# WhatAShot/Electrocardio-Panorama

Measured on AMD Instinct MI355X. Metric: ECG-samples/sec (train step), higher is better.
Workload: dtype f32 (conv products: fp32 operands split into fp16 hi+lo = 22-23 bits, block-scaled, 3 fp16 matrix products each, fp32 accumulate; fp32-class, not IEEE fp32)

## Files before the change

### electrocardio_panorama_amd/csrc/elementwise.hip

```cpp
#include "nef_common.h"
#include "roi_unpool.h"

namespace {

__global__ void chscale_fwd_kernel(const float* __restrict__ x, const float* __restrict__ s, int64_t s_bs,
                                   float* __restrict__ y, int B, int C, int T) {
    const int64_t rows = (int64_t)B * C;
    const int wave = threadIdx.x >> 6, lane = threadIdx.x & 63;
    for (int64_t row = (int64_t)blockIdx.x * 4 + wave; row < rows; row += (int64_t)gridDim.x * 4) {
        const int b = (int)(row / C), c = (int)(row % C);
        const float f = s[(int64_t)b * s_bs + c];
        const float* xr = x + row * T;
        float* yr = y + row * T;
        for (int t = lane; t < T; t += 64) yr[t] = xr[t] * f;
    }
}

__global__ void chscale_bwd_kernel(const float* __restrict__ gy, const float* __restrict__ x,
                                   const float* __restrict__ s, int64_t s_bs, float* __restrict__ gx,
                                   float* __restrict__ gs, int B, int C, int T, int relu_x) {
    const int64_t rows = (int64_t)B * C;
    const int wave = threadIdx.x >> 6, lane = threadIdx.x & 63;
    for (int64_t row = (int64_t)blockIdx.x * 4 + wave; row < rows; row += (int64_t)gridDim.x * 4) {
        const int b = (int)(row / C), c = (int)(row % C);
// ... 145 lines not shown
            lat[t] = m0;
            lat[t + 64] = m1;
            d0[t] = f * m0;
            d0[t + 64] = f * m1;
            d0[pass + t] = f * p0;
            d0[pass + t + 64] = f * p1;
        }
        for (; t < TW; t += 64) {
            vec s = src[t];
            vec pk = s;
            for (int v = 1; v < V; ++v) {
                const vec x = src[(int64_t)v * lead + t];
                s += x;
                if (v == cp) pk = x;
            }
            const vec m = s / fv;
            lat[t] = m;
            d0[t] = f * m;
            d0[pass + t] = f * pk;
        }
    }
}

__global__ __launch_bounds__(256) void lead_mean_mix_shared_pair_kernel(const float* __restrict__ z1, const float* __restrict__ z2r,
                                                                        const float* __restrict__ q, float* __restrict__ latent,
                                                                        float* __restrict__ D2, int B, int V, int T, int c1, int c2,
                                                                        const int32_t* __restrict__ choice_dev, int cshift) {
    typedef float vec __attribute__((ext_vector_type(4)));
    if (choice_dev) { c1 = choice_dev[0]; c2 = choice_dev[1]; }
    const int64_t pairs = (int64_t)B * 128;
    const int pshift = cshift - 1;
    const int64_t nidx = (int64_t)B << pshift;
    const int wave = threadIdx.x >> 6, lane = threadIdx.x & 63;
    const float fv = (float)V;
    const int TW = T / 2;
    const int mid = T / 4;
    const int64_t pass = pairs * TW;
    const int64_t lead = (int64_t)128 * T / 4;
    for (int64_t idx = (int64_t)blockIdx.x * 4 + wave; idx < nidx; idx += (int64_t)gridDim.x * 4) {
        const int64_t pr = ((idx >> pshift) << 7) | (idx & ((1 << pshift) - 1));
        const int64_t row = 2 * pr;
        const int b = (int)(row >> 8), c = (int)(row & 255);
        const vec* src = (const vec*)((c < 128 ? z1 : z2r) + ((int64_t)b * V * 128 + (c & 127)) * T);
        const int cp = c < 128 ? c1 : c2;
        const float f0 = q[row], f1 = q[row + 1];
        vec* lat = (vec*)latent + pr * TW;
        vec* d0 = (vec*)D2 + pr * TW;
        int t = lane;
        for (; t + 64 < TW; t += 128) {
            vec s0 = src[t], s1 = src[t + 64];
            vec p0 = s0, p1 = s1;
            for (int v = 1; v < V; ++v) {
                const vec x0 = src[(int64_t)v * lead + t], x1 = src[(int64_t)v * lead + t + 64];
                s0 += x0;
                s1 += x1;
                if (v == cp) { p0 = x0; p1 = x1; }
            }
            const vec m0 = s0 / fv, m1 = s1 / fv;
            const vec g0 = t < mid ? vec{f0, f0, f0, f0} : (t > mid ? vec{f1, f1, f1, f1} : vec{f0, f0, f1, f1});
            const vec g1 = t + 64 < mid ? vec{f0, f0, f0, f0} : (t + 64 > mid ? vec{f1, f1, f1, f1} : vec{f0, f0, f1, f1});
            lat[t] = m0;
            lat[t + 64] = m1;
            d0[t] = g0 * m0;
            d0[t + 64] = g1 * m1;
            d0[pass + t] = g0 * p0;
            d0[pass + t + 64] = g1 * p1;
        }
        for (; t < TW; t += 64) {
            vec sm = src[t];
            vec pk = sm;
            for (int v = 1; v < V; ++v) {
                const vec x = src[(int64_t)v * lead + t];
                sm += x;
                if (v == cp) pk = x;
            }
            const vec m = sm / fv;
            const vec g0 = t < mid ? vec{f0, f0, f0, f0} : (t > mid ? vec{f1, f1, f1, f1} : vec{f0, f0, f1, f1});
            lat[t] = m;
            d0[t] = g0 * m;
            d0[pass + t] = g0 * pk;
        }
    }
}

__device__ __forceinline__ float up2_bwd_edge(const float* __restrict__ gr, int Tin, int m) {
    const int To = 2 * Tin;
    float s = 0.f;
#pragma unroll
    for (int d = -1; d <= 2; ++d) {
        const int i = 2 * m + d;
        if (i < 0 || i >= To) continue;
        float src = 0.5f * ((float)i + 0.5f) - 0.5f;
        if (src < 0.f) src = 0.f;
        int i0 = (int)src;
        if (i0 > Tin - 1) i0 = Tin - 1;
        const int i1 = i0 + (i0 < Tin - 1 ? 1 : 0);
        const float l1 = src - (float)i0;
        const float l0 = 1.f - l1;
        const float g = gr[i];
        if (i0 == m) s += l0 * g;
        if (i1 == m) s += l1 * g;
    }
    return s;
}

// ... 76 lines not shown
            } else {
                ga = g0[t]; gb = g0[gpass + t]; gc = SHARED ? 0.f : g0[2 * gpass + t];
            }
            const float g_pick = SHARED ? gb : (first ? gb : gc);
            const float g_mean = SHARED ? ga : (first ? (ga + gc) : (ga + gb));
            const float l = lat[t];
            const float pk = zsrc[(int64_t)pick_v * 128 * T + t];
            acc += g_mean * l + g_pick * pk;
            const float gm = f * g_mean / fv;
            for (int v = 0; v < V; ++v) {
                float o = gm + (v == pick_v ? f * g_pick : 0.f);
                if (relu_z1 && first && !(zsrc[(int64_t)v * 128 * T + t] > 0.f)) o = 0.f;
                gdst[(int64_t)v * 128 * T + t] = o;
            }
        }
        acc = nef_wave_sum(acc);
        if (lane == 0) gq[row] = acc;
    }
}

constexpr int MIX_RS_MAX_V = 4;

template <int NV>
__global__ __launch_bounds__(256) void mix_bwd_shared_pair_kernel(const float* __restrict__ gD, const float* __restrict__ latent,
                                                                  const float* __restrict__ z1, const float* __restrict__ z2r,
                                                                  const float* __restrict__ q, float* __restrict__ gz1,
                                                                  float* __restrict__ gz2r, float* __restrict__ gq, int B, int V, int T,
                                                                  int c1, int c2, const int32_t* __restrict__ choice_dev, int relu_z1,
                                                                  int cshift, double* __restrict__ rowsum) {
    typedef float vec __attribute__((ext_vector_type(4)));
    if (choice_dev) { c1 = choice_dev[0]; c2 = choice_dev[1]; }
    const int64_t pairs = (int64_t)B * 128;
    const int pshift = cshift - 1;
    const int64_t nidx = (int64_t)B << pshift;
    const int wave = threadIdx.x >> 6, lane = threadIdx.x & 63;
    const float fv = (float)V;
    const int TW = T / 2, mid = T / 4;
    const int64_t gpass = pairs * TW;
    const int64_t lead = (int64_t)128 * T / 4;
    for (int64_t idx = (int64_t)blockIdx.x * 4 + wave; idx < nidx; idx += (int64_t)gridDim.x * 4) {
        const int64_t pr = ((idx >> pshift) << 7) | (idx & ((1 << pshift) - 1));
        const int64_t row = 2 * pr;
        const int b = (int)(row >> 8), c = (int)(row & 255);
        const bool first = c < 128;
        const int pick_v = first ? c1 : c2;
        const float f0 = q[row], f1 = q[row + 1];
        const vec* lat = (const vec*)latent + pr * TW;
        const vec* zsrc = (const vec*)((first ? z1 : z2r) + ((int64_t)b * V * 128 + (c & 127)) * T);
        vec* gdst = (vec*)((first ? gz1 : gz2r) + ((int64_t)b * V * 128 + (c & 127)) * T);
        const vec* g0 = (const vec*)gD + pr * TW;
        const vec* g1r = g0 + gpass;
        const bool mask = relu_z1 && first;
        float acc0 = 0.f, acc1 = 0.f;
        double rs0[NV > 0 ? NV : 1], rs1[NV > 0 ? NV : 1];
#pragma unroll
        for (int v = 0; v < NV; ++v) rs0[v] = rs1[v] = 0.0;
        for (int t = lane; t < TW; t += 64) {
            const vec ga = g0[t], gb = g1r[t], l4 = lat[t], pk = zsrc[(int64_t)pick_v * lead + t];
            const vec fq = t < mid ? vec{f0, f0, f0, f0} : (t > mid ? vec{f1, f1, f1, f1} : vec{f0, f0, f1, f1});
#pragma unroll
            for (int e = 0; e < 4; ++e) {
                const float term = ga[e] * l4[e] + gb[e] * pk[e];
                if (t < mid || (t == mid && e < 2)) acc0 += term; else acc1 += term;
// ... 18 lines not shown
                        const vec o = one_lead(v);
                        const double lo = (double)o[0] + (double)o[1], hi = (double)o[2] + (double)o[3];
                        if (t < mid) rs0[v] += lo + hi;
                        else if (t > mid) rs1[v] += lo + hi;
                        else { rs0[v] += lo; rs1[v] += hi; }
                    }
            } else {
                for (int v = 0; v < V; ++v) one_lead(v);
            }
        }
        acc0 = nef_wave_sum(acc0);
        acc1 = nef_wave_sum(acc1);
        if (lane == 0) { gq[row] = acc0; gq[row + 1] = acc1; }
        if constexpr (NV > 0) {
            double* const rdst = rowsum + (int64_t)b * V * 128 + (c & 127);
#pragma unroll
            for (int v = 0; v < NV; ++v)
                if (v < V) {
                    const double a0 = nef_wave_sum_d(rs0[v]), a1 = nef_wave_sum_d(rs1[v]);
                    if (lane == 0) { rdst[v * 128] = a0; rdst[v * 128 + 1] = a1; }
                }
        }
    }
}

__device__ __forceinline__ float up2_at(const float* __restrict__ xr, int Tin, int i) {
    float src = 0.5f * ((float)i + 0.5f) - 0.5f;
    if (src < 0.f) src = 0.f;
    int i0 = (int)src;
    if (i0 > Tin - 1) i0 = Tin - 1;
    const int i1 = i0 + (i0 < Tin - 1 ? 1 : 0);
    const float l1 = src - (float)i0;
    const float l0 = 1.f - l1;
    return l0 * xr[i0] + l1 * xr[i1];
}

__global__ void upsample2_fwd_kernel(const float* __restrict__ x, float* __restrict__ y, int64_t N, int Tin) {
    const int To = 2 * Tin;
    const int wave = threadIdx.x >> 6, lane = threadIdx.x & 63;
    for (int64_t row = (int64_t)blockIdx.x * 4 + wave; row < N; row += (int64_t)gridDim.x * 4) {
        const float* xr = x + row * Tin;
        float* yr = y + row * To;
        for (int i = lane; i < To; i += 64) yr[i] = up2_at(xr, Tin, i);
    }
}

// ... 1965 lines not shown
                           q, latent, D2, B, V, T, c1, c2, choice_dev, cshift);
    else if (T % 2 == 0)
        hipLaunchKernelGGL(lead_mean_mix_shared_kernel<2>, grid, dim3(256), 0, st, z1, z2r, q, latent, D2, B, V, T, c1, c2, choice_dev,
                           cshift);
    else
        hipLaunchKernelGGL(lead_mean_mix_shared_kernel<1>, grid, dim3(256), 0, st, z1, z2r, q, latent, D2, B, V, T, c1, c2, choice_dev,
                           cshift);
}

int nef_lead_mean_mix_shared(const float* z1, const float* z2r, const float* q, float* latent, float* D2, int B, int V,
                             int T, int c1, int c2, const int32_t* choice_dev, nef_stream_t stream) {
    NEF_ENTER();
    NEF_REQUIRE(z1 && z2r && q && latent && D2, NEF_E_NULL);
    NEF_REQUIRE(B > 0 && V > 0 && T > 0 && c1 >= 0 && c1 < V && c2 >= 0 && c2 < V, NEF_E_SHAPE);
    lead_mean_mix_shared_launch(z1, z2r, q, latent, D2, B, V, T, c1, c2, choice_dev, 8, NEF_ST);
    return nef_launch_status();
}

int nef_lead_mean_mix_unpool(const float* z1, const float* z2b, const int64_t* rois, const float* q, float* latent, float* D2,
                             int32_t* status, int B, int V, int T, int c1, int c2, const int32_t* choice_dev, nef_stream_t stream) {
    NEF_ENTER();
    NEF_REQUIRE(z1 && z2b && rois && q && latent && D2, NEF_E_NULL);
    NEF_REQUIRE(B > 0 && V > 0 && V <= NEF_UNPOOL_MIX_MAX_V && T > 0 && c1 >= 0 && c1 < V && c2 >= 0 && c2 < V, NEF_E_SHAPE);
    lead_mean_mix_shared_launch(z1, nullptr, q, latent, D2, B, V, T, c1, c2, choice_dev, 7, NEF_ST);
    nef_unpool_mix_fwd_z2(z2b, rois, q, latent, D2, status, B, V, T, c2, choice_dev, NEF_ST);
    return nef_launch_status();
}

int nef_mix_bwd(const float* gD, const float* latent, const float* z1, const float* z2r, const float* q, float* gz1,
                float* gz2r, float* gq, int B, int V, int T, int c1, int c2, const int32_t* choice_dev, int relu_z1, int up,
                int shared, nef_stream_t stream) {
    NEF_ENTER();
    NEF_REQUIRE(gD && latent && z1 && z2r && q && gz1 && gz2r && gq, NEF_E_NULL);
    NEF_REQUIRE(B > 0 && V > 0 && T > (shared ? 1 : 0) && c1 >= 0 && c1 < V && c2 >= 0 && c2 < V, NEF_E_SHAPE);
    const bool al16 = (((uintptr_t)gD | (uintptr_t)latent | (uintptr_t)z1 | (uintptr_t)z2r | (uintptr_t)gz1 | (uintptr_t)gz2r) & 15) == 0;
#define NEF_MIX_BWD(UP, SHARED)                                                                                                \
    hipLaunchKernelGGL((mix_bwd_kernel<UP, SHARED>), dim3(nef_stream_grid((int64_t)B * 256, 4)), dim3(256), 0, NEF_ST, gD, latent, \
                       z1, z2r, q, gz1, gz2r, gq, B, V, T, c1, c2, choice_dev, relu_z1, 8)
    if (shared && !up && T % 4 == 2 && T >= 8 && al16)
        hipLaunchKernelGGL(mix_bwd_shared_pair_kernel<0>, dim3(nef_stream_grid((int64_t)B * 128, 4)), dim3(256), 0, NEF_ST, gD, latent, z1,
                           z2r, q, gz1, gz2r, gq, B, V, T, c1, c2, choice_dev, relu_z1, 8, (double*)nullptr);
    else if (shared && up) NEF_MIX_BWD(true, true);
    else if (shared) NEF_MIX_BWD(false, true);
    else if (up) NEF_MIX_BWD(true, false);
    else NEF_MIX_BWD(false, false);
#undef NEF_MIX_BWD
    return nef_launch_status();
}

static int mix_bwd_unpool_launch(const float* gD, const float* latent, const float* z1, const float* z2b, const int64_t* rois, const float* q,
                                 float* gz1, float* gz2b, float* gq, int B, int V, int T, int c1, int c2, const int32_t* choice_dev,
                                 int relu_z1, float* gz1_chan_sum, void* ws, size_t ws_bytes, int* in_kernel, nef_stream_t stream) {
    NEF_REQUIRE(gD && latent && z1 && z2b && rois && q && gz1 && gz2b && gq, NEF_E_NULL);
    NEF_REQUIRE(B > 0 && V > 0 && T > 1 && T <= NEF_UNPOOL_MIX_MAX_T && c1 >= 0 && c1 < V && c2 >= 0 && c2 < V, NEF_E_SHAPE);
    const bool al16 = (((uintptr_t)gD | (uintptr_t)latent | (uintptr_t)z1 | (uintptr_t)gz1) & 15) == 0;
    const bool pair = T % 4 == 2 && T >= 8 && al16;
    const bool rs = gz1_chan_sum && pair && V <= MIX_RS_MAX_V;
    if (in_kernel) *in_kernel = rs;
#define NEF_MIX_PAIR(NV, ROWSUM)                                                                                                        \
    hipLaunchKernelGGL(mix_bwd_shared_pair_kernel<NV>, dim3(nef_stream_grid((int64_t)B * 64, 4)), dim3(256), 0, NEF_ST, gD, latent, z1, \
                       (const float*)nullptr, q, gz1, (float*)nullptr, gq, B, V, T, c1, c2, choice_dev, relu_z1, 7, ROWSUM)
    if (rs) {
        NEF_MIX_PAIR(MIX_RS_MAX_V, (double*)ws);
        hipLaunchKernelGGL(rowsum_to_channel, dim3(128 * V), dim3(256), 0, NEF_ST, (const double*)ws, gz1_chan_sum, B, 128 * V);
    } else if (pair)
        NEF_MIX_PAIR(0, (double*)nullptr);
    else
        hipLaunchKernelGGL((mix_bwd_kernel<false, true>), dim3(nef_stream_grid((int64_t)B * 128, 4)), dim3(256), 0, NEF_ST, gD, latent, z1,
                           (const float*)nullptr, q, gz1, (float*)nullptr, gq, B, V, T, c1, c2, choice_dev, relu_z1, 7);
#undef NEF_MIX_PAIR
    nef_unpool_mix_bwd_z2(gD, latent, z2b, rois, q, gz2b, gq, B, V, T, c2, choice_dev, pair ? 4 : ((T & 1) == 0 && T >= 8 ? 2 : 1), NEF_ST);
    if (gz1_chan_sum && !rs)
        return nef_chan_sum(gz1, gz1_chan_sum, ws, ws_bytes, B, 128 * V, T, stream);
    return nef_launch_status();
}

int nef_mix_bwd_unpool(const float* gD, const float* latent, const float* z1, const float* z2b, const int64_t* rois, const float* q,
                       float* gz1, float* gz2b, float* gq, int B, int V, int T, int c1, int c2, const int32_t* choice_dev, int relu_z1,
                       nef_stream_t stream) {
    NEF_ENTER();
    return mix_bwd_unpool_launch(gD, latent, z1, z2b, rois, q, gz1, gz2b, gq, B, V, T, c1, c2, choice_dev, relu_z1, nullptr, nullptr, 0,
                                 nullptr, stream);
}

size_t nef_mix_bwd_unpool_rs_ws_bytes(int B, int V) {
    if (B <= 0 || V <= 0) return 0;
    const size_t rows = (size_t)B * 128 * V * sizeof(double), cs = nef_chan_sum_ws_bytes(128 * V);
    return rows > cs ? rows : cs;
}

int nef_mix_bwd_unpool_rs(const float* gD, const float* latent, const float* z1, const float* z2b, const int64_t* rois, const float* q,
                          float* gz1, float* gz2b, float* gq, float* gz1_chan_sum, void* ws, size_t ws_bytes, int* in_kernel, int B, int V,
                          int T, int c1, int c2, const int32_t* choice_dev, int relu_z1, nef_stream_t stream) {
    NEF_ENTER();
// ... 579 lines not shown
```

### electrocardio_panorama_amd/csrc/roi.hip

```cpp
#include "nef_common.h"
#include "roi_unpool.h"

namespace {

using namespace nef_unpool;

__device__ __forceinline__ float grid_x(const int64_t* __restrict__ roi_b, int j, int s, int T) {
    const float sc = (float)(2.0 / (double)T);
    const float r0 = ((float)roi_b[2 * j] * 0.25f) * sc + (-1.0f);
    const float r1 = ((float)roi_b[2 * j + 1] * 0.25f) * sc + (-1.0f);
    const float step = (r1 - r0) / (float)(BINS - 1);
    return s < BINS / 2 ? r0 + step * (float)s : r1 - step * (float)(BINS - 1 - s);
}

__device__ __forceinline__ float col_weight(float gx) {
    const float ix = ((gx + 1.f) * 1.f - 1.f) * 0.5f;
    const float x0 = floorf(ix);
    const float we = ix - x0;
    const float ww = 1.f - we;
    float w = 0.f;
    if (x0 == 0.f) w += ww;
    if (x0 + 1.f == 0.f) w += we;
    return w;
}
// ... 121 lines not shown
            constexpr int NU = 20;
            for (int t0 = 0; t0 < T; t0 += 64 * NU) {
                float v[NU];
#pragma unroll
                for (int u = 0; u < NU; ++u) v[u] = (t0 + u * 64 + lane < T) ? grow[t0 + u * 64 + lane] : 0.f;
#pragma unroll
                for (int u = 0; u < NU; ++u)
                    if (t0 + u * 64 + lane < T) strip[t0 + u * 64 + lane] = v[u];
            }
            __builtin_amdgcn_fence(__ATOMIC_RELEASE, "wavefront");
            __builtin_amdgcn_wave_barrier();
            gr = strip;
        }
        float* gz = gzseg + row * NSEG * SEGW;
        float acc[(NSEG + 1) / 2] = {0.f, 0.f, 0.f, 0.f};
        unpool_gather_row(gr, st, lane, acc);
#pragma unroll
        for (int k = 0; k < (NSEG + 1) / 2; ++k)
            if (2 * k + half < NSEG) gz[(2 * k + half) * SEGW + s] = acc[k];
        if constexpr (STAGED) __builtin_amdgcn_wave_barrier();
    }
}

__device__ __forceinline__ bool segment_of(const SegTable& st, int t, int& i, float& sc, int& jb) {
    int off = st.off[0];
    sc = st.scale[0];
    jb = 0;
#pragma unroll
    for (int j = 1; j < NSEG; ++j)
        if (t >= st.off[j]) { off = st.off[j]; sc = st.scale[j]; jb = j * SEGW; }
    i = t - off;
    return t < st.off[NSEG - 1] + st.len[NSEG - 1];
}

template <int W>
__global__ __launch_bounds__(256) void unpool_mix_fwd_z2_kernel(const float* __restrict__ z2b, const int64_t* __restrict__ rois,
                                                                const float* __restrict__ q, float* __restrict__ latent,
                                                                float* __restrict__ D2, int32_t* __restrict__ status, int B, int V,
                                                                int T, int c2, const int32_t* __restrict__ choice_dev) {
    typedef float vec __attribute__((ext_vector_type(W)));
    extern __shared__ float strip_lds[];
    constexpr int ROW = NSEG * SEGW;
    if (choice_dev) c2 = choice_dev[1];
    const int64_t rows = (int64_t)B * 128;
    const int wave = __builtin_amdgcn_readfirstlane((int)(threadIdx.x >> 6)), lane = threadIdx.x & 63;
    const int64_t per_wave = (rows + (int64_t)gridDim.x * 4 - 1) / ((int64_t)gridDim.x * 4);
    const int64_t row_lo = ((int64_t)blockIdx.x * 4 + wave) * per_wave;
    const int64_t row_hi = row_lo + per_wave < rows ? row_lo + per_wave : rows;
    float* strip = strip_lds + wave * V * ROW;
    const int n = V * ROW;
    const float fv = (float)V;
    const int64_t pass = (int64_t)B * 256 * T;
    int b_cur = -1;
    SegTable st;
    for (int64_t row = row_lo; row < row_hi; ++row) {
        const int b = (int)(row >> 7), c = (int)(row & 127);
        if (b != b_cur) {
            b_cur = b;
            const bool ok = load_segments(rois + (int64_t)b * NSEG * 2, T, st);
            if (!ok && status && lane == 0) status[0] = 1;
        }
        const float* zr = z2b + ((int64_t)b * V * 128 + c) * ROW;
        constexpr int NU = 8;
        for (int e0 = 0; e0 < n; e0 += 64 * NU) {
            float r[NU];
#pragma unroll
            for (int u = 0; u < NU; ++u) {
                const int e = e0 + u * 64 + lane, v = e / ROW;
                r[u] = e < n ? zr[(int64_t)v * 128 * ROW + (e - v * ROW)] : 0.f;
            }
#pragma unroll
            for (int u = 0; u < NU; ++u)
                if (e0 + u * 64 + lane < n) strip[e0 + u * 64 + lane] = r[u];
        }
        __builtin_amdgcn_fence(__ATOMIC_RELEASE, "wavefront");
        __builtin_amdgcn_wave_barrier();
        const int64_t orow = ((int64_t)b * 256 + 128 + c) * T;
        const float f = q[b * 256 + 128 + c];
        for (int p = lane; p < T / W; p += 64) {
            vec m, dm, dp;
#pragma unroll
            for (int w = 0; w < W; ++w) {
                int i, jb;
                float sc;
                const bool in = segment_of(st, W * p + w, i, sc, jb);
                int i0 = 0, i1 = 0;
                float l0 = 0.f, l1 = 0.f;
                if (in) lerp_src(i, sc, i0, i1, l0, l1);
                float sum = 0.f, pk = 0.f;
                for (int v = 0; v < V; ++v) {
                    const float val = in ? unpool_lerp(l0, strip[v * ROW + jb + i0], l1, strip[v * ROW + jb + i1]) : 0.f;
                    sum = v == 0 ? val : sum + val;
                    if (v == 0 || v == c2) pk = val;
                }
                const float mean = sum / fv;
                m[w] = mean;
                dm[w] = f * mean;
                dp[w] = f * pk;
            }
            *(vec*)(latent + orow + W * p) = m;
            *(vec*)(D2 + orow + W * p) = dm;
            *(vec*)(D2 + pass + orow + W * p) = dp;
        }
        __builtin_amdgcn_wave_barrier();
    }
}

template <int G>
__global__ __launch_bounds__(256) void unpool_mix_bwd_z2_kernel(const float* __restrict__ gD, const float* __restrict__ latent,
                                                                const float* __restrict__ z2b, const int64_t* __restrict__ rois,
                                                                const float* __restrict__ q, float* __restrict__ gz2b,
                                                                float* __restrict__ gq, int B, int V, int T, int c2,
                                                                const int32_t* __restrict__ choice_dev) {
    extern __shared__ float strip_lds[];
    constexpr int ROW = NSEG * SEGW;
    if (choice_dev) c2 = choice_dev[1];
    const int64_t rows = (int64_t)B * 128;
    const int wave = __builtin_amdgcn_readfirstlane((int)(threadIdx.x >> 6)), lane = threadIdx.x & 63;
    const int s = lane & (SEGW - 1), half = lane >> 5;
    const int64_t per_wave = (rows + (int64_t)gridDim.x * 4 - 1) / ((int64_t)gridDim.x * 4);
    const int64_t row_lo = ((int64_t)blockIdx.x * 4 + wave) * per_wave;
    const int64_t row_hi = row_lo + per_wave < rows ? row_lo + per_wave : rows;
    float* sa = strip_lds + wave * (2 * T + ROW);
    float* sb = sa + T;
    float* pick = sb + T;
    const float fv = (float)V;
    const int64_t pass = (int64_t)B * 256 * T;
    int b_cur = -1;
    SegTable st;
    for (int64_t row = row_lo; row < row_hi; ++row) {
        const int b = (int)(row >> 7), c = (int)(row & 127);
        if (b != b_cur) {
            b_cur = b;
            load_segments(rois + (int64_t)b * NSEG * 2, T, st);
        }
        const float* zr = z2b + (((int64_t)b * V + c2) * 128 + c) * ROW;
#pragma unroll
        for (int u = 0; u < 4; ++u)
            if (u * 64 + lane < ROW) pick[u * 64 + lane] = zr[u * 64 + lane];
        __builtin_amdgcn_fence(__ATOMIC_RELEASE, "wavefront");
        __builtin_amdgcn_wave_barrier();
        const int64_t grow = ((int64_t)b * 256 + 128 + c) * T;
        const float f = q[b * 256 + 128 + c];
        float acc = 0.f;
        constexpr int NU = G == 4 ? 6 : (G == 2 ? 10 : 20);
        const int shift = G == 4 ? (c & 1) * T : 0;
        const int kb = shift / G, ke = (shift + T + G - 1) / G;
        for (int k0 = (kb & ~63) + lane; k0 < ke; k0 += 64 * NU) {
            float ga[NU][G], gb[NU][G], la[NU][G];
#pragma unroll
            for (int u = 0; u < NU; ++u) {
                const int k = k0 + 64 * u;
                if constexpr (G == 1) {
                    const bool in = k >= kb && k < ke;
                    ga[u][0] = in ? gD[grow + k] : 0.f;
                    gb[u][0] = in ? gD[pass + grow + k] : 0.f;
                    la[u][0] = in ? latent[grow + k] : 0.f;
                } else {
#pragma unroll
                    for (int e = 0; e < G; e += 2) {
                        const int t = G * k + e - shift;
                        const bool in = k >= kb && k < ke && t >= 0 && t < T;
                        const nef_f32x2 z = {0.f, 0.f};
                        const nef_f32x2 a2 = in ? *(const nef_f32x2*)(gD + grow + t) : z;
                        const nef_f32x2 b2 = in ? *(const nef_f32x2*)(gD + pass + grow + t) : z;
                        const nef_f32x2 l2 = in ? *(const nef_f32x2*)(latent + grow + t) : z;
                        ga[u][e] = a2[0], ga[u][e + 1] = a2[1];
                        gb[u][e] = b2[0], gb[u][e + 1] = b2[1];
                        la[u][e] = l2[0], la[u][e + 1] = l2[1];
                    }
                }
            }
#pragma unroll
            for (int u = 0; u < NU; ++u) {
                const int k = k0 + 64 * u;
#pragma unroll
                for (int e = 0; e < G; ++e) {
                    const int t = G * k + e - shift;
                    if (k >= kb && k < ke && t >= 0 && t < T) {
                        int i, jb, i0, i1;
                        float sc, l0, l1, pk = 0.f;
                        if (segment_of(st, t, i, sc, jb)) {
                            lerp_src(i, sc, i0, i1, l0, l1);
                            pk = unpool_lerp(l0, pick[jb + i0], l1, pick[jb + i1]);
                        }
                        acc += ga[u][e] * la[u][e] + gb[u][e] * pk;
                        const float gm = f * ga[u][e] / fv;
                        sa[t] = gm + 0.f;
                        sb[t] = gm + f * gb[u][e];
                    }
                }
            }
        }
        __builtin_amdgcn_fence(__ATOMIC_RELEASE, "wavefront");
        __builtin_amdgcn_wave_barrier();
        float ra[(NSEG + 1) / 2] = {0.f, 0.f, 0.f, 0.f}, rb[(NSEG + 1) / 2] = {0.f, 0.f, 0.f, 0.f};
        unpool_gather_row(sa, st, lane, ra);
        unpool_gather_row(sb, st, lane, rb);
        for (int v = 0; v < V; ++v) {
            float* gz = gz2b + (((int64_t)b * V + v) * 128 + c) * ROW;
#pragma unroll
            for (int k = 0; k < (NSEG + 1) / 2; ++k)
                if (2 * k + half < NSEG) gz[(2 * k + half) * SEGW + s] = v == c2 ? rb[k] : ra[k];
        }
        acc = nef_wave_sum(acc);
        if (lane == 0) gq[b * 256 + 128 + c] = acc;
        __builtin_amdgcn_wave_barrier();
    }
}

__global__ void roi_segment_table_kernel(const int64_t* __restrict__ rois, int64_t* __restrict__ seg_start,
                                         int64_t* __restrict__ seg_len, int n) {
    const int i = blockIdx.x * blockDim.x + threadIdx.x;
    if (i >= n) return;
    const int64_t a = latent_index(rois[2 * i]);
    const int64_t e = latent_index(rois[2 * i + 1]);
    seg_start[i] = a;
    seg_len[i] = e - a;
}

}

void nef_unpool_mix_fwd_z2(const float* z2b, const int64_t* rois, const float* q, float* latent, float* D2, int32_t* status, int B,
                           int V, int T, int c2, const int32_t* choice_dev, hipStream_t st) {
    const dim3 grid(nef_stream_grid((int64_t)B * 128, 4));
    const size_t lds = (size_t)4 * V * NSEG * SEGW * sizeof(float);
    const bool al8 = (((uintptr_t)latent | (uintptr_t)D2) & 7) == 0;
    if (T % 2 == 0 && al8)
        hipLaunchKernelGGL(unpool_mix_fwd_z2_kernel<2>, grid, dim3(256), lds, st, z2b, rois, q, latent, D2, status, B, V, T, c2,
                           choice_dev);
    else
        hipLaunchKernelGGL(unpool_mix_fwd_z2_kernel<1>, grid, dim3(256), lds, st, z2b, rois, q, latent, D2, status, B, V, T, c2,
                           choice_dev);
}

void nef_unpool_mix_bwd_z2(const float* gD, const float* latent, const float* z2b, const int64_t* rois, const float* q, float* gz2b,
                           float* gq, int B, int V, int T, int c2, const int32_t* choice_dev, int group, hipStream_t st) {
    static_assert((size_t)4 * (2 * NEF_UNPOOL_MIX_MAX_T + NSEG * SEGW) * sizeof(float) <= 65536, "four waves' strips fit the default LDS limit");
    const size_t lds = (size_t)4 * (2 * T + NSEG * SEGW) * sizeof(float);
    const dim3 grid(nef_stream_grid((int64_t)B * 128, 4));
    if (group == 4)
        hipLaunchKernelGGL(unpool_mix_bwd_z2_kernel<4>, grid, dim3(256), lds, st, gD, latent, z2b, rois, q, gz2b, gq, B, V, T, c2, choice_dev);
    else if (group == 2)
        hipLaunchKernelGGL(unpool_mix_bwd_z2_kernel<2>, grid, dim3(256), lds, st, gD, latent, z2b, rois, q, gz2b, gq, B, V, T, c2, choice_dev);
    else
        hipLaunchKernelGGL(unpool_mix_bwd_z2_kernel<1>, grid, dim3(256), lds, st, gD, latent, z2b, rois, q, gz2b, gq, B, V, T, c2, choice_dev);
}

#define NEF_ST ((hipStream_t)stream)

extern "C" {

static bool window_covers_taps(int T, int zT, int t_off) {
    const int r0 = (T - 1) / 2, r1 = (r0 + 1 < T) ? r0 + 1 : r0;
    return zT > 0 && t_off >= 0 && t_off <= r0 && r1 < t_off + zT && t_off + zT <= T;
}

int nef_roi_align_fwd(const float* z, const int64_t* rois, float* out, int B, int C, int T, int zT, int t_off,
                      nef_stream_t stream) {
    NEF_ENTER();
    NEF_REQUIRE(z && rois && out, NEF_E_NULL);
    NEF_REQUIRE(B > 0 && C > 0 && T > 0 && window_covers_taps(T, zT, t_off), NEF_E_SHAPE);
    const int64_t n = (int64_t)B * C * NSEG * BINS;
    hipLaunchKernelGGL(roi_align_fwd_kernel, dim3(nef_stream_grid(n, 256)), dim3(256), 0, NEF_ST, z, rois, out, B, C, T,
                       zT, t_off);
    return nef_launch_status();
// ... 48 lines not shown
```

### electrocardio_panorama_amd/csrc/roi_unpool.h

```cpp
#pragma once
#include "nef_common.h"

namespace nef_unpool {

constexpr int NSEG = NEF_N_SEG;
constexpr int BINS = NEF_ROI_BINS;
constexpr int SEGW = 2 * NEF_ROI_BINS;

__device__ __forceinline__ int64_t latent_index(int64_t roi) {
    return (int64_t)((float)roi * 0.25f);
}

struct SegTable { int start[NSEG]; int len[NSEG]; int off[NSEG]; float scale[NSEG]; };

__device__ __forceinline__ bool load_segments(const int64_t* __restrict__ roi_b, int T, SegTable& st) {
    int run = 0;
    bool ok = true;
#pragma unroll
    for (int j = 0; j < NSEG; ++j) {
        const int64_t a = latent_index(roi_b[2 * j]);
        const int64_t e = latent_index(roi_b[2 * j + 1]);
        int64_t len = e - a;
        if (len < 0) { ok = false; len = 0; }
        if (run + len > T) { ok = false; len = T - run; }
// ... 57 lines not shown
            const int b0 = unpool_first_reaching(s, len, sc, (float)len * (1.f / SEGW));
            const int nb = __shfl_down(b0, 1), pb = __shfl_up(b0, 1);
            const int b1 = s + 1 < SEGW ? nb : len;
            const int a0 = s > 0 ? pb : b0;
            const float* gp = gr + off;
            float fi = (float)a0 + 0.5f;
            const float sm1 = (float)(s - 1);
            for (int i = a0; i < b0; ++i, fi += 1.f) {
                float src = sc * fi - 0.5f;
                src = src < 0.f ? 0.f : src;
                acc += (src - sm1) * gp[i];
            }
            const float c0 = s == SEGW - 1 ? 1.f : (float)(s + 1), k = s == SEGW - 1 ? 0.f : 1.f;
            for (int i = b0; i < b1; ++i, fi += 1.f) {
                float src = sc * fi - 0.5f;
                src = src < 0.f ? 0.f : src;
                acc += (c0 - k * src) * gp[i];
            }
        }
        acc_out[jj >> 1] = acc;
    }
}

}

NEF_HIDDEN void nef_unpool_mix_fwd_z2(const float* z2b, const int64_t* rois, const float* q, float* latent, float* D2, int32_t* status,
                                      int B, int V, int T, int c2, const int32_t* choice_dev, hipStream_t st);
NEF_HIDDEN void nef_unpool_mix_bwd_z2(const float* gD, const float* latent, const float* z2b, const int64_t* rois, const float* q,
                                      float* gz2b, float* gq, int B, int V, int T, int c2, const int32_t* choice_dev, int group,
                                      hipStream_t st);
```

Before: 10050.

## Fuse z1 lead-mean mix and z2 unpool mix into one heterogeneous-wave kernel

Wraps the shared-pair mix and the ROI-unpool z2 mix bodies as device functions and launches one kernel per direction in which some waves handle the z2 unpool rows and the others handle the z1 pair rows. This removes a separate launch and lets the two independent halves run concurrently on the GPU instead of back to back. In exchange, the combined kernel uses more LDS and registers per block and fixes the wave split between the two kinds of work, which can unbalance them.

```diff
diff --git a/electrocardio_panorama_amd/csrc/elementwise.hip b/electrocardio_panorama_amd/csrc/elementwise.hip
--- a/electrocardio_panorama_amd/csrc/elementwise.hip
+++ b/electrocardio_panorama_amd/csrc/elementwise.hip
@@ -191,22 +191,20 @@
     }
 }
 
-__global__ __launch_bounds__(256) void lead_mean_mix_shared_pair_kernel(const float* __restrict__ z1, const float* __restrict__ z2r,
-                                                                        const float* __restrict__ q, float* __restrict__ latent,
-                                                                        float* __restrict__ D2, int B, int V, int T, int c1, int c2,
-                                                                        const int32_t* __restrict__ choice_dev, int cshift) {
+__device__ __forceinline__ void lead_mean_mix_shared_pair_rows(const float* __restrict__ z1, const float* __restrict__ z2r,
+                                                               const float* __restrict__ q, float* __restrict__ latent,
+                                                               float* __restrict__ D2, int B, int V, int T, int c1, int c2, int cshift,
+                                                               int64_t idx0, int64_t stride, int lane) {
     typedef float vec __attribute__((ext_vector_type(4)));
-    if (choice_dev) { c1 = choice_dev[0]; c2 = choice_dev[1]; }
     const int64_t pairs = (int64_t)B * 128;
     const int pshift = cshift - 1;
     const int64_t nidx = (int64_t)B << pshift;
-    const int wave = threadIdx.x >> 6, lane = threadIdx.x & 63;
     const float fv = (float)V;
     const int TW = T / 2;
     const int mid = T / 4;
     const int64_t pass = pairs * TW;
     const int64_t lead = (int64_t)128 * T / 4;
-    for (int64_t idx = (int64_t)blockIdx.x * 4 + wave; idx < nidx; idx += (int64_t)gridDim.x * 4) {
+    for (int64_t idx = idx0; idx < nidx; idx += stride) {
         const int64_t pr = ((idx >> pshift) << 7) | (idx & ((1 << pshift) - 1));
         const int64_t row = 2 * pr;
         const int b = (int)(row >> 8), c = (int)(row & 255);
@@ -250,6 +248,37 @@
             d0[pass + t] = g0 * pk;
         }
     }
+}
+
+__global__ __launch_bounds__(256) void lead_mean_mix_shared_pair_kernel(const float* __restrict__ z1, const float* __restrict__ z2r,
+                                                                        const float* __restrict__ q, float* __restrict__ latent,
+                                                                        float* __restrict__ D2, int B, int V, int T, int c1, int c2,
+                                                                        const int32_t* __restrict__ choice_dev, int cshift) {
+    if (choice_dev) { c1 = choice_dev[0]; c2 = choice_dev[1]; }
+    const int wave = threadIdx.x >> 6, lane = threadIdx.x & 63;
+    lead_mean_mix_shared_pair_rows(z1, z2r, q, latent, D2, B, V, T, c1, c2, cshift, (int64_t)blockIdx.x * 4 + wave, (int64_t)gridDim.x * 4,
+                                   lane);
+}
+
+constexpr int MIX_ONE_FWD_W = 4, MIX_ONE_BWD_W = 2;
+
+template <int W1, int W2>
+__global__ __launch_bounds__(64 * (W1 + W2)) void lead_mean_mix_unpool_pair_kernel(const float* __restrict__ z1, const float* __restrict__ z2b,
+                                                                                   const int64_t* __restrict__ rois,
+                                                                                   const float* __restrict__ q, float* __restrict__ latent,
+                                                                                   float* __restrict__ D2, int32_t* __restrict__ status,
+                                                                                   int B, int V, int T, int c1, int c2,
+                                                                                   const int32_t* __restrict__ choice_dev) {
+    extern __shared__ float strip_lds[];
+    if (choice_dev) { c1 = choice_dev[0]; c2 = choice_dev[1]; }
+    const int wave = __builtin_amdgcn_readfirstlane((int)(threadIdx.x >> 6)), lane = threadIdx.x & 63;
+    if (wave < W2)
+        nef_unpool::unpool_mix_fwd_z2_rows<2>(z2b, rois, q, latent, D2, status, B, V, T, c2,
+                                              strip_lds + wave * V * nef_unpool::NSEG * nef_unpool::SEGW,
+                                              (int64_t)blockIdx.x * W2 + wave, (int64_t)gridDim.x * W2, lane);
+    else
+        lead_mean_mix_shared_pair_rows(z1, nullptr, q, latent, D2, B, V, T, c1, c2, 7, (int64_t)blockIdx.x * W1 + (wave - W2),
+                                       (int64_t)gridDim.x * W1, lane);
 }
 
 __device__ __forceinline__ float up2_bwd_edge(const float* __restrict__ gr, int Tin, int m) {
@@ -372,23 +401,21 @@
 constexpr int MIX_RS_MAX_V = 4;
 
 template <int NV>
-__global__ __launch_bounds__(256) void mix_bwd_shared_pair_kernel(const float* __restrict__ gD, const float* __restrict__ latent,
-                                                                  const float* __restrict__ z1, const float* __restrict__ z2r,
-                                                                  const float* __restrict__ q, float* __restrict__ gz1,
-                                                                  float* __restrict__ gz2r, float* __restrict__ gq, int B, int V, int T,
-                                                                  int c1, int c2, const int32_t* __restrict__ choice_dev, int relu_z1,
-                                                                  int cshift, double* __restrict__ rowsum) {
+__device__ __forceinline__ void mix_bwd_shared_pair_rows(const float* __restrict__ gD, const float* __restrict__ latent,
+                                                         const float* __restrict__ z1, const float* __restrict__ z2r,
+                                                         const float* __restrict__ q, float* __restrict__ gz1,
+                                                         float* __restrict__ gz2r, float* __restrict__ gq, int B, int V, int T,
+                                                         int c1, int c2, int relu_z1, int cshift, double* __restrict__ rowsum,
+                                                         int64_t idx0, int64_t stride, int lane) {
     typedef float vec __attribute__((ext_vector_type(4)));
-    if (choice_dev) { c1 = choice_dev[0]; c2 = choice_dev[1]; }
     const int64_t pairs = (int64_t)B * 128;
     const int pshift = cshift - 1;
     const int64_t nidx = (int64_t)B << pshift;
-    const int wave = threadIdx.x >> 6, lane = threadIdx.x & 63;
     const float fv = (float)V;
     const int TW = T / 2, mid = T / 4;
     const int64_t gpass = pairs * TW;
     const int64_t lead = (int64_t)128 * T / 4;
-    for (int64_t idx = (int64_t)blockIdx.x * 4 + wave; idx < nidx; idx += (int64_t)gridDim.x * 4) {
+    for (int64_t idx = idx0; idx < nidx; idx += stride) {
         const int64_t pr = ((idx >> pshift) << 7) | (idx & ((1 << pshift) - 1));
         const int64_t row = 2 * pr;
         const int b = (int)(row >> 8), c = (int)(row & 255);
@@ -453,6 +480,39 @@
                 }
         }
     }
+}
+
+template <int NV>
+__global__ __launch_bounds__(256) void mix_bwd_shared_pair_kernel(const float* __restrict__ gD, const float* __restrict__ latent,
+                                                                  const float* __restrict__ z1, const float* __restrict__ z2r,
+                                                                  const float* __restrict__ q, float* __restrict__ gz1,
+                                                                  float* __restrict__ gz2r, float* __restrict__ gq, int B, int V, int T,
+                                                                  int c1, int c2, const int32_t* __restrict__ choice_dev, int relu_z1,
+                                                                  int cshift, double* __restrict__ rowsum) {
+    if (choice_dev) { c1 = choice_dev[0]; c2 = choice_dev[1]; }
+    const int wave = threadIdx.x >> 6, lane = threadIdx.x & 63;
+    mix_bwd_shared_pair_rows<NV>(gD, latent, z1, z2r, q, gz1, gz2r, gq, B, V, T, c1, c2, relu_z1, cshift, rowsum,
+                                 (int64_t)blockIdx.x * 4 + wave, (int64_t)gridDim.x * 4, lane);
+}
+
+template <int NV, int W1, int W2>
+__global__ __launch_bounds__(64 * (W1 + W2)) void mix_bwd_unpool_pair_kernel(const float* __restrict__ gD, const float* __restrict__ latent,
+                                                                             const float* __restrict__ z1, const float* __restrict__ z2b,
+                                                                             const int64_t* __restrict__ rois, const float* __restrict__ q,
+                                                                             float* __restrict__ gz1, float* __restrict__ gz2b,
+                                                                             float* __restrict__ gq, int B, int V, int T, int c1, int c2,
+                                                                             const int32_t* __restrict__ choice_dev, int relu_z1,
+                                                                             double* __restrict__ rowsum) {
+    extern __shared__ float strip_lds[];
+    if (choice_dev) { c1 = choice_dev[0]; c2 = choice_dev[1]; }
+    const int wave = __builtin_amdgcn_readfirstlane((int)(threadIdx.x >> 6)), lane = threadIdx.x & 63;
+    if (wave < W2)
+        nef_unpool::unpool_mix_bwd_z2_rows<4>(gD, latent, z2b, rois, q, gz2b, gq, B, V, T, c2,
+                                              strip_lds + wave * (2 * T + nef_unpool::NSEG * nef_unpool::SEGW),
+                                              (int64_t)blockIdx.x * W2 + wave, (int64_t)gridDim.x * W2, lane);
+    else
+        mix_bwd_shared_pair_rows<NV>(gD, latent, z1, nullptr, q, gz1, nullptr, gq, B, V, T, c1, c2, relu_z1, 7, rowsum,
+                                     (int64_t)blockIdx.x * W1 + (wave - W2), (int64_t)gridDim.x * W1, lane);
 }
 
 __device__ __forceinline__ float up2_at(const float* __restrict__ xr, int Tin, int i) {
@@ -2464,6 +2524,14 @@
     NEF_ENTER();
     NEF_REQUIRE(z1 && z2b && rois && q && latent && D2, NEF_E_NULL);
     NEF_REQUIRE(B > 0 && V > 0 && V <= NEF_UNPOOL_MIX_MAX_V && T > 0 && c1 >= 0 && c1 < V && c2 >= 0 && c2 < V, NEF_E_SHAPE);
+    constexpr int W = MIX_ONE_FWD_W;
+    const bool al16 = (((uintptr_t)z1 | (uintptr_t)latent | (uintptr_t)D2) & 15) == 0;
+    const size_t lds = (size_t)W * V * NEF_N_SEG * 2 * NEF_ROI_BINS * sizeof(float);
+    if (T % 4 == 2 && al16 && lds <= 65536) {
+        hipLaunchKernelGGL((lead_mean_mix_unpool_pair_kernel<W, W>), dim3(nef_stream_grid((int64_t)B * 64, W)), dim3(128 * W), lds, NEF_ST, z1,
+                           z2b, rois, q, latent, D2, status, B, V, T, c1, c2, choice_dev);
+        return nef_launch_status();
+    }
     lead_mean_mix_shared_launch(z1, nullptr, q, latent, D2, B, V, T, c1, c2, choice_dev, 7, NEF_ST);
     nef_unpool_mix_fwd_z2(z2b, rois, q, latent, D2, status, B, V, T, c2, choice_dev, NEF_ST);
     return nef_launch_status();
@@ -2499,19 +2567,23 @@
     const bool pair = T % 4 == 2 && T >= 8 && al16;
     const bool rs = gz1_chan_sum && pair && V <= MIX_RS_MAX_V;
     if (in_kernel) *in_kernel = rs;
-#define NEF_MIX_PAIR(NV, ROWSUM)                                                                                                        \
-    hipLaunchKernelGGL(mix_bwd_shared_pair_kernel<NV>, dim3(nef_stream_grid((int64_t)B * 64, 4)), dim3(256), 0, NEF_ST, gD, latent, z1, \
-                       (const float*)nullptr, q, gz1, (float*)nullptr, gq, B, V, T, c1, c2, choice_dev, relu_z1, 7, ROWSUM)
-    if (rs) {
-        NEF_MIX_PAIR(MIX_RS_MAX_V, (double*)ws);
-        hipLaunchKernelGGL(rowsum_to_channel, dim3(128 * V), dim3(256), 0, NEF_ST, (const double*)ws, gz1_chan_sum, B, 128 * V);
-    } else if (pair)
-        NEF_MIX_PAIR(0, (double*)nullptr);
-    else
+    if (pair) {
+        constexpr int W = MIX_ONE_BWD_W;
+        static_assert((size_t)W * (2 * NEF_UNPOOL_MIX_MAX_T + NEF_N_SEG * 2 * NEF_ROI_BINS) * sizeof(float) <= 65536, "the z2 waves' strips fit the default LDS limit");
+        const dim3 grid(nef_stream_grid((int64_t)B * 64, W));
+        const size_t lds = (size_t)W * (2 * T + NEF_N_SEG * 2 * NEF_ROI_BINS) * sizeof(float);
+        if (rs) {
+            hipLaunchKernelGGL((mix_bwd_unpool_pair_kernel<MIX_RS_MAX_V, W, W>), grid, dim3(128 * W), lds, NEF_ST, gD, latent, z1, z2b, rois, q,
+                               gz1, gz2b, gq, B, V, T, c1, c2, choice_dev, relu_z1, (double*)ws);
+            hipLaunchKernelGGL(rowsum_to_channel, dim3(128 * V), dim3(256), 0, NEF_ST, (const double*)ws, gz1_chan_sum, B, 128 * V);
+        } else
+            hipLaunchKernelGGL((mix_bwd_unpool_pair_kernel<0, W, W>), grid, dim3(128 * W), lds, NEF_ST, gD, latent, z1, z2b, rois, q, gz1,
+                               gz2b, gq, B, V, T, c1, c2, choice_dev, relu_z1, (double*)nullptr);
+    } else {
         hipLaunchKernelGGL((mix_bwd_kernel<false, true>), dim3(nef_stream_grid((int64_t)B * 128, 4)), dim3(256), 0, NEF_ST, gD, latent, z1,
                            (const float*)nullptr, q, gz1, (float*)nullptr, gq, B, V, T, c1, c2, choice_dev, relu_z1, 7);
-#undef NEF_MIX_PAIR
-    nef_unpool_mix_bwd_z2(gD, latent, z2b, rois, q, gz2b, gq, B, V, T, c2, choice_dev, pair ? 4 : ((T & 1) == 0 && T >= 8 ? 2 : 1), NEF_ST);
+        nef_unpool_mix_bwd_z2(gD, latent, z2b, rois, q, gz2b, gq, B, V, T, c2, choice_dev, (T & 1) == 0 && T >= 8 ? 2 : 1, NEF_ST);
+    }
     if (gz1_chan_sum && !rs)
         return nef_chan_sum(gz1, gz1_chan_sum, ws, ws_bytes, B, 128 * V, T, stream);
     return nef_launch_status();
diff --git a/electrocardio_panorama_amd/csrc/roi.hip b/electrocardio_panorama_amd/csrc/roi.hip
--- a/electrocardio_panorama_amd/csrc/roi.hip
+++ b/electrocardio_panorama_amd/csrc/roi.hip
@@ -167,88 +167,16 @@
     }
 }
 
-__device__ __forceinline__ bool segment_of(const SegTable& st, int t, int& i, float& sc, int& jb) {
-    int off = st.off[0];
-    sc = st.scale[0];
-    jb = 0;
-#pragma unroll
-    for (int j = 1; j < NSEG; ++j)
-        if (t >= st.off[j]) { off = st.off[j]; sc = st.scale[j]; jb = j * SEGW; }
-    i = t - off;
-    return t < st.off[NSEG - 1] + st.len[NSEG - 1];
-}
-
 template <int W>
 __global__ __launch_bounds__(256) void unpool_mix_fwd_z2_kernel(const float* __restrict__ z2b, const int64_t* __restrict__ rois,
                                                                 const float* __restrict__ q, float* __restrict__ latent,
                                                                 float* __restrict__ D2, int32_t* __restrict__ status, int B, int V,
                                                                 int T, int c2, const int32_t* __restrict__ choice_dev) {
-    typedef float vec __attribute__((ext_vector_type(W)));
     extern __shared__ float strip_lds[];
-    constexpr int ROW = NSEG * SEGW;
     if (choice_dev) c2 = choice_dev[1];
-    const int64_t rows = (int64_t)B * 128;
-    const int wave = __builtin_amdgcn_readfirstlane((int)(threadIdx.x >> 6)), lane = threadIdx.x & 63;
-    const int64_t per_wave = (rows + (int64_t)gridDim.x * 4 - 1) / ((int64_t)gridDim.x * 4);
-    const int64_t row_lo = ((int64_t)blockIdx.x * 4 + wave) * per_wave;
-    const int64_t row_hi = row_lo + per_wave < rows ? row_lo + per_wave : rows;
-    float* strip = strip_lds + wave * V * ROW;
-    const int n = V * ROW;
-    const float fv = (float)V;
-    const int64_t pass = (int64_t)B * 256 * T;
-    int b_cur = -1;
-    SegTable st;
-    for (int64_t row = row_lo; row < row_hi; ++row) {
-        const int b = (int)(row >> 7), c = (int)(row & 127);
-        if (b != b_cur) {
-            b_cur = b;
-            const bool ok = load_segments(rois + (int64_t)b * NSEG * 2, T, st);
-            if (!ok && status && lane == 0) status[0] = 1;
-        }
-        const float* zr = z2b + ((int64_t)b * V * 128 + c) * ROW;
-        constexpr int NU = 8;
-        for (int e0 = 0; e0 < n; e0 += 64 * NU) {
-            float r[NU];
-#pragma unroll
-            for (int u = 0; u < NU; ++u) {
-                const int e = e0 + u * 64 + lane, v = e / ROW;
-                r[u] = e < n ? zr[(int64_t)v * 128 * ROW + (e - v * ROW)] : 0.f;
-            }
-#pragma unroll
-            for (int u = 0; u < NU; ++u)
-                if (e0 + u * 64 + lane < n) strip[e0 + u * 64 + lane] = r[u];
-        }
-        __builtin_amdgcn_fence(__ATOMIC_RELEASE, "wavefront");
-        __builtin_amdgcn_wave_barrier();
-        const int64_t orow = ((int64_t)b * 256 + 128 + c) * T;
-        const float f = q[b * 256 + 128 + c];
-        for (int p = lane; p < T / W; p += 64) {
-            vec m, dm, dp;
-#pragma unroll
-            for (int w = 0; w < W; ++w) {
-                int i, jb;
-                float sc;
-                const bool in = segment_of(st, W * p + w, i, sc, jb);
-                int i0 = 0, i1 = 0;
-                float l0 = 0.f, l1 = 0.f;
-                if (in) lerp_src(i, sc, i0, i1, l0, l1);
-                float sum = 0.f, pk = 0.f;
-                for (int v = 0; v < V; ++v) {
-                    const float val = in ? unpool_lerp(l0, strip[v * ROW + jb + i0], l1, strip[v * ROW + jb + i1]) : 0.f;
-                    sum = v == 0 ? val : sum + val;
-                    if (v == 0 || v == c2) pk = val;
-                }
-                const float mean = sum / fv;
-                m[w] = mean;
-                dm[w] = f * mean;
-                dp[w] = f * pk;
-            }
-            *(vec*)(latent + orow + W * p) = m;
-            *(vec*)(D2 + orow + W * p) = dm;
-            *(vec*)(D2 + pass + orow + W * p) = dp;
-        }
-        __builtin_amdgcn_wave_barrier();
-    }
+    const int wave = __builtin_amdgcn_readfirstlane((int)(threadIdx.x >> 6)), lane = threadIdx.x & 63;
+    unpool_mix_fwd_z2_rows<W>(z2b, rois, q, latent, D2, status, B, V, T, c2, strip_lds + wave * V * NSEG * SEGW,
+                              (int64_t)blockIdx.x * 4 + wave, (int64_t)gridDim.x * 4, lane);
 }
 
 template <int G>
@@ -258,100 +186,10 @@
                                                                 float* __restrict__ gq, int B, int V, int T, int c2,
                                                                 const int32_t* __restrict__ choice_dev) {
     extern __shared__ float strip_lds[];
-    constexpr int ROW = NSEG * SEGW;
     if (choice_dev) c2 = choice_dev[1];
-    const int64_t rows = (int64_t)B * 128;
-    const int wave = __builtin_amdgcn_readfirstlane((int)(threadIdx.x >> 6)), lane = threadIdx.x & 63;
-    const int s = lane & (SEGW - 1), half = lane >> 5;
-    const int64_t per_wave = (rows + (int64_t)gridDim.x * 4 - 1) / ((int64_t)gridDim.x * 4);
-    const int64_t row_lo = ((int64_t)blockIdx.x * 4 + wave) * per_wave;
-    const int64_t row_hi = row_lo + per_wave < rows ? row_lo + per_wave : rows;
-    float* sa = strip_lds + wave * (2 * T + ROW);
-    float* sb = sa + T;
-    float* pick = sb + T;
-    const float fv = (float)V;
-    const int64_t pass = (int64_t)B * 256 * T;
-    int b_cur = -1;
-    SegTable st;
-    for (int64_t row = row_lo; row < row_hi; ++row) {
-        const int b = (int)(row >> 7), c = (int)(row & 127);
-        if (b != b_cur) {
-            b_cur = b;
-            load_segments(rois + (int64_t)b * NSEG * 2, T, st);
-        }
-        const float* zr = z2b + (((int64_t)b * V + c2) * 128 + c) * ROW;
-#pragma unroll
-        for (int u = 0; u < 4; ++u)
-            if (u * 64 + lane < ROW) pick[u * 64 + lane] = zr[u * 64 + lane];
-        __builtin_amdgcn_fence(__ATOMIC_RELEASE, "wavefront");
-        __builtin_amdgcn_wave_barrier();
-        const int64_t grow = ((int64_t)b * 256 + 128 + c) * T;
-        const float f = q[b * 256 + 128 + c];
-        float acc = 0.f;
-        constexpr int NU = G == 4 ? 6 : (G == 2 ? 10 : 20);
-        const int shift = G == 4 ? (c & 1) * T : 0;
-        const int kb = shift / G, ke = (shift + T + G - 1) / G;
-        for (int k0 = (kb & ~63) + lane; k0 < ke; k0 += 64 * NU) {
-            float ga[NU][G], gb[NU][G], la[NU][G];
-#pragma unroll
-            for (int u = 0; u < NU; ++u) {
-                const int k = k0 + 64 * u;
-                if constexpr (G == 1) {
-                    const bool in = k >= kb && k < ke;
-                    ga[u][0] = in ? gD[grow + k] : 0.f;
-                    gb[u][0] = in ? gD[pass + grow + k] : 0.f;
-                    la[u][0] = in ? latent[grow + k] : 0.f;
-                } else {
-#pragma unroll
-                    for (int e = 0; e < G; e += 2) {
-                        const int t = G * k + e - shift;
-                        const bool in = k >= kb && k < ke && t >= 0 && t < T;
-                        const nef_f32x2 z = {0.f, 0.f};
-                        const nef_f32x2 a2 = in ? *(const nef_f32x2*)(gD + grow + t) : z;
-                        const nef_f32x2 b2 = in ? *(const nef_f32x2*)(gD + pass + grow + t) : z;
-                        const nef_f32x2 l2 = in ? *(const nef_f32x2*)(latent + grow + t) : z;
-                        ga[u][e] = a2[0], ga[u][e + 1] = a2[1];
-                        gb[u][e] = b2[0], gb[u][e + 1] = b2[1];
-                        la[u][e] = l2[0], la[u][e + 1] = l2[1];
-                    }
-                }
-            }
-#pragma unroll
-            for (int u = 0; u < NU; ++u) {
-                const int k = k0 + 64 * u;
-#pragma unroll
-                for (int e = 0; e < G; ++e) {
-                    const int t = G * k + e - shift;
-                    if (k >= kb && k < ke && t >= 0 && t < T) {
-                        int i, jb, i0, i1;
-                        float sc, l0, l1, pk = 0.f;
-                        if (segment_of(st, t, i, sc, jb)) {
-                            lerp_src(i, sc, i0, i1, l0, l1);
-                            pk = unpool_lerp(l0, pick[jb + i0], l1, pick[jb + i1]);
-                        }
-                        acc += ga[u][e] * la[u][e] + gb[u][e] * pk;
-                        const float gm = f * ga[u][e] / fv;
-                        sa[t] = gm + 0.f;
-                        sb[t] = gm + f * gb[u][e];
-                    }
-                }
-            }
-        }
-        __builtin_amdgcn_fence(__ATOMIC_RELEASE, "wavefront");
-        __builtin_amdgcn_wave_barrier();
-        float ra[(NSEG + 1) / 2] = {0.f, 0.f, 0.f, 0.f}, rb[(NSEG + 1) / 2] = {0.f, 0.f, 0.f, 0.f};
-        unpool_gather_row(sa, st, lane, ra);
-        unpool_gather_row(sb, st, lane, rb);
-        for (int v = 0; v < V; ++v) {
-            float* gz = gz2b + (((int64_t)b * V + v) * 128 + c) * ROW;
-#pragma unroll
-            for (int k = 0; k < (NSEG + 1) / 2; ++k)
-                if (2 * k + half < NSEG) gz[(2 * k + half) * SEGW + s] = v == c2 ? rb[k] : ra[k];
-        }
-        acc = nef_wave_sum(acc);
-        if (lane == 0) gq[b * 256 + 128 + c] = acc;
-        __builtin_amdgcn_wave_barrier();
-    }
+    const int wave = __builtin_amdgcn_readfirstlane((int)(threadIdx.x >> 6)), lane = threadIdx.x & 63;
+    unpool_mix_bwd_z2_rows<G>(gD, latent, z2b, rois, q, gz2b, gq, B, V, T, c2, strip_lds + wave * (2 * T + NSEG * SEGW),
+                              (int64_t)blockIdx.x * 4 + wave, (int64_t)gridDim.x * 4, lane);
 }
 
 __global__ void roi_segment_table_kernel(const int64_t* __restrict__ rois, int64_t* __restrict__ seg_start,
@@ -384,9 +222,7 @@
     static_assert((size_t)4 * (2 * NEF_UNPOOL_MIX_MAX_T + NSEG * SEGW) * sizeof(float) <= 65536, "four waves' strips fit the default LDS limit");
     const size_t lds = (size_t)4 * (2 * T + NSEG * SEGW) * sizeof(float);
     const dim3 grid(nef_stream_grid((int64_t)B * 128, 4));
-    if (group == 4)
-        hipLaunchKernelGGL(unpool_mix_bwd_z2_kernel<4>, grid, dim3(256), lds, st, gD, latent, z2b, rois, q, gz2b, gq, B, V, T, c2, choice_dev);
-    else if (group == 2)
+    if (group == 2)
         hipLaunchKernelGGL(unpool_mix_bwd_z2_kernel<2>, grid, dim3(256), lds, st, gD, latent, z2b, rois, q, gz2b, gq, B, V, T, c2, choice_dev);
     else
         hipLaunchKernelGGL(unpool_mix_bwd_z2_kernel<1>, grid, dim3(256), lds, st, gD, latent, z2b, rois, q, gz2b, gq, B, V, T, c2, choice_dev);
diff --git a/electrocardio_panorama_amd/csrc/roi_unpool.h b/electrocardio_panorama_amd/csrc/roi_unpool.h
--- a/electrocardio_panorama_amd/csrc/roi_unpool.h
+++ b/electrocardio_panorama_amd/csrc/roi_unpool.h
@@ -103,6 +103,187 @@
     }
 }
 
+__device__ __forceinline__ bool segment_of(const SegTable& st, int t, int& i, float& sc, int& jb) {
+    int off = st.off[0];
+    sc = st.scale[0];
+    jb = 0;
+#pragma unroll
+    for (int j = 1; j < NSEG; ++j)
+        if (t >= st.off[j]) { off = st.off[j]; sc = st.scale[j]; jb = j * SEGW; }
+    i = t - off;
+    return t < st.off[NSEG - 1] + st.len[NSEG - 1];
+}
+
+
+template <int W>
+__device__ __forceinline__ void unpool_mix_fwd_z2_rows(const float* __restrict__ z2b, const int64_t* __restrict__ rois,
+                                                       const float* __restrict__ q, float* __restrict__ latent,
+                                                       float* __restrict__ D2, int32_t* __restrict__ status, int B, int V, int T,
+                                                       int c2, float* strip, int64_t wave_id, int64_t n_waves, int lane) {
+    typedef float vec __attribute__((ext_vector_type(W)));
+    constexpr int ROW = NSEG * SEGW;
+    const int64_t rows = (int64_t)B * 128;
+    const int64_t per_wave = (rows + n_waves - 1) / n_waves;
+    const int64_t row_lo = wave_id * per_wave;
+    const int64_t row_hi = row_lo + per_wave < rows ? row_lo + per_wave : rows;
+    const int n = V * ROW;
+    const float fv = (float)V;
+    const int64_t pass = (int64_t)B * 256 * T;
+    int b_cur = -1;
+    SegTable st;
+    for (int64_t row = row_lo; row < row_hi; ++row) {
+        const int b = (int)(row >> 7), c = (int)(row & 127);
+        if (b != b_cur) {
+            b_cur = b;
+            const bool ok = load_segments(rois + (int64_t)b * NSEG * 2, T, st);
+            if (!ok && status && lane == 0) status[0] = 1;
+        }
+        const float* zr = z2b + ((int64_t)b * V * 128 + c) * ROW;
+        constexpr int NU = 8;
+        for (int e0 = 0; e0 < n; e0 += 64 * NU) {
+            float r[NU];
+#pragma unroll
+            for (int u = 0; u < NU; ++u) {
+                const int e = e0 + u * 64 + lane, v = e / ROW;
+                r[u] = e < n ? zr[(int64_t)v * 128 * ROW + (e - v * ROW)] : 0.f;
+            }
+#pragma unroll
+            for (int u = 0; u < NU; ++u)
+                if (e0 + u * 64 + lane < n) strip[e0 + u * 64 + lane] = r[u];
+        }
+        __builtin_amdgcn_fence(__ATOMIC_RELEASE, "wavefront");
+        __builtin_amdgcn_wave_barrier();
+        const int64_t orow = ((int64_t)b * 256 + 128 + c) * T;
+        const float f = q[b * 256 + 128 + c];
+        for (int p = lane; p < T / W; p += 64) {
+            vec m, dm, dp;
+#pragma unroll
+            for (int w = 0; w < W; ++w) {
+                int i, jb;
+                float sc;
+                const bool in = segment_of(st, W * p + w, i, sc, jb);
+                int i0 = 0, i1 = 0;
+                float l0 = 0.f, l1 = 0.f;
+                if (in) lerp_src(i, sc, i0, i1, l0, l1);
+                float sum = 0.f, pk = 0.f;
+                for (int v = 0; v < V; ++v) {
+                    const float val = in ? unpool_lerp(l0, strip[v * ROW + jb + i0], l1, strip[v * ROW + jb + i1]) : 0.f;
+                    sum = v == 0 ? val : sum + val;
+                    if (v == 0 || v == c2) pk = val;
+                }
+                const float mean = sum / fv;
+                m[w] = mean;
+                dm[w] = f * mean;
+                dp[w] = f * pk;
+            }
+            *(vec*)(latent + orow + W * p) = m;
+            *(vec*)(D2 + orow + W * p) = dm;
+            *(vec*)(D2 + pass + orow + W * p) = dp;
+        }
+        __builtin_amdgcn_wave_barrier();
+    }
+}
+
+template <int G>
+__device__ __forceinline__ void unpool_mix_bwd_z2_rows(const float* __restrict__ gD, const float* __restrict__ latent,
+                                                       const float* __restrict__ z2b, const int64_t* __restrict__ rois,
+                                                       const float* __restrict__ q, float* __restrict__ gz2b,
+                                                       float* __restrict__ gq, int B, int V, int T, int c2, float* strip,
+                                                       int64_t wave_id, int64_t n_waves, int lane) {
+    constexpr int ROW = NSEG * SEGW;
+    const int64_t rows = (int64_t)B * 128;
+    const int s = lane & (SEGW - 1), half = lane >> 5;
+    const int64_t per_wave = (rows + n_waves - 1) / n_waves;
+    const int64_t row_lo = wave_id * per_wave;
+    const int64_t row_hi = row_lo + per_wave < rows ? row_lo + per_wave : rows;
+    float* sa = strip;
+    float* sb = sa + T;
+    float* pick = sb + T;
+    const float fv = (float)V;
+    const int64_t pass = (int64_t)B * 256 * T;
+    int b_cur = -1;
+    SegTable st;
+    for (int64_t row = row_lo; row < row_hi; ++row) {
+        const int b = (int)(row >> 7), c = (int)(row & 127);
+        if (b != b_cur) {
+            b_cur = b;
+            load_segments(rois + (int64_t)b * NSEG * 2, T, st);
+        }
+        const float* zr = z2b + (((int64_t)b * V + c2) * 128 + c) * ROW;
+#pragma unroll
+        for (int u = 0; u < 4; ++u)
+            if (u * 64 + lane < ROW) pick[u * 64 + lane] = zr[u * 64 + lane];
+        __builtin_amdgcn_fence(__ATOMIC_RELEASE, "wavefront");
+        __builtin_amdgcn_wave_barrier();
+        const int64_t grow = ((int64_t)b * 256 + 128 + c) * T;
+        const float f = q[b * 256 + 128 + c];
+        float acc = 0.f;
+        constexpr int NU = G == 4 ? 6 : (G == 2 ? 10 : 20);
+        const int shift = G == 4 ? (c & 1) * T : 0;
+        const int kb = shift / G, ke = (shift + T + G - 1) / G;
+        for (int k0 = (kb & ~63) + lane; k0 < ke; k0 += 64 * NU) {
+            float ga[NU][G], gb[NU][G], la[NU][G];
+#pragma unroll
+            for (int u = 0; u < NU; ++u) {
+                const int k = k0 + 64 * u;
+                if constexpr (G == 1) {
+                    const bool in = k >= kb && k < ke;
+                    ga[u][0] = in ? gD[grow + k] : 0.f;
+                    gb[u][0] = in ? gD[pass + grow + k] : 0.f;
+                    la[u][0] = in ? latent[grow + k] : 0.f;
+                } else {
+#pragma unroll
+                    for (int e = 0; e < G; e += 2) {
+                        const int t = G * k + e - shift;
+                        const bool in = k >= kb && k < ke && t >= 0 && t < T;
+                        const nef_f32x2 z = {0.f, 0.f};
+                        const nef_f32x2 a2 = in ? *(const nef_f32x2*)(gD + grow + t) : z;
+                        const nef_f32x2 b2 = in ? *(const nef_f32x2*)(gD + pass + grow + t) : z;
+                        const nef_f32x2 l2 = in ? *(const nef_f32x2*)(latent + grow + t) : z;
+                        ga[u][e] = a2[0], ga[u][e + 1] = a2[1];
+                        gb[u][e] = b2[0], gb[u][e + 1] = b2[1];
+                        la[u][e] = l2[0], la[u][e + 1] = l2[1];
+                    }
+                }
+            }
+#pragma unroll
+            for (int u = 0; u < NU; ++u) {
+                const int k = k0 + 64 * u;
+#pragma unroll
+                for (int e = 0; e < G; ++e) {
+                    const int t = G * k + e - shift;
+                    if (k >= kb && k < ke && t >= 0 && t < T) {
+                        int i, jb, i0, i1;
+                        float sc, l0, l1, pk = 0.f;
+                        if (segment_of(st, t, i, sc, jb)) {
+                            lerp_src(i, sc, i0, i1, l0, l1);
+                            pk = unpool_lerp(l0, pick[jb + i0], l1, pick[jb + i1]);
+                        }
+                        acc += ga[u][e] * la[u][e] + gb[u][e] * pk;
+                        const float gm = f * ga[u][e] / fv;
+                        sa[t] = gm + 0.f;
+                        sb[t] = gm + f * gb[u][e];
+                    }
+                }
+            }
+        }
+        __builtin_amdgcn_fence(__ATOMIC_RELEASE, "wavefront");
+        __builtin_amdgcn_wave_barrier();
+        float ra[(NSEG + 1) / 2] = {0.f, 0.f, 0.f, 0.f}, rb[(NSEG + 1) / 2] = {0.f, 0.f, 0.f, 0.f};
+        unpool_gather_row(sa, st, lane, ra);
+        unpool_gather_row(sb, st, lane, rb);
+        for (int v = 0; v < V; ++v) {
+            float* gz = gz2b + (((int64_t)b * V + v) * 128 + c) * ROW;
+#pragma unroll
+            for (int k = 0; k < (NSEG + 1) / 2; ++k)
+                if (2 * k + half < NSEG) gz[(2 * k + half) * SEGW + s] = v == c2 ? rb[k] : ra[k];
+        }
+        acc = nef_wave_sum(acc);
+        if (lane == 0) gq[b * 256 + 128 + c] = acc;
+        __builtin_amdgcn_wave_barrier();
+    }
+}
+
 }
 
 NEF_HIDDEN void nef_unpool_mix_fwd_z2(const float* z2b, const int64_t* rois, const float* q, float* latent, float* D2, int32_t* status,
```

Measured after the change: 10090, median of 6. Within noise of the previous version (+0.4%).
